# IC3Net/IC3Net

Measured on NVIDIA H100. Metric: agent-env-steps/sec, higher is better.
Workload: dtype f32

## Files before the change

ic3net_b200/_lib.py:

```python
import ctypes as C
import os

import torch

_HERE = os.path.dirname(os.path.abspath(__file__))
LIB_PATH = os.path.join(_HERE, "libic3net_b200.so")

MAX_AGENTS = 32
MAX_HEADS = 4
MAX_HEAD_DIM = 16
MAX_PASSES = 4
CELL_LSTM, CELL_TANH = 0, 1
LSTM_IMG_BYTES = 786432

ERR_EPISODE_DONE = 1
ERR_ROUTE_OVERRUN = 2
ERR_BAD_ACTION = 4
ERR_PIPELINE = 0x100
ERR_FP16_RANGE = 0x200

PP_MODES = {"mixed": 0, "cooperative": 1, "competitive": 2}

_p = C.c_void_p

# ... 52 lines not shown
    _fields_ = [("enc_wT", _p), ("enc_b", _p), ("c_wT", _p), ("c_b", _p), ("lstm_wT", _p), ("lstm_b", _p),
                ("head_w", _p), ("head_b", _p), ("lstm_img", _p), ("bias_cat", _p), ("f_wT", _p), ("f_b", _p), ("flags", _p)]


class PolicyIO(C.Structure):
    _fields_ = [("x", _p), ("h", _p), ("c", _p), ("comm_action", _p), ("alive", _p), ("fresh", _p), ("tick", _p),
                ("draws", _p), ("h_out", _p), ("c_out", _p), ("value", _p), ("logp", _p), ("action", _p),
                ("workspace", _p), ("err", _p), ("pp_env", _p), ("pp_state", _p), ("tj_env", _p), ("tj_state", _p),
                ("x_table", _p), ("defer_heads", C.c_int32), ("pass_index", C.c_int32)]


class BpttPlan(C.Structure):
    _fields_ = [("cfg", C.POINTER(PolicyCfg)), ("w", C.POINTER(PolicyPacked)), ("pp_env", C.POINTER(PPCfg)),
                ("tj_env", C.POINTER(TJCfg)), ("x_table", _p), ("value_coeff", C.c_float), ("entr", C.c_float),
                ("workspace", _p)]


class BpttStepIO(C.Structure):
    _fields_ = [("t", C.c_int32), ("reserved0", C.c_int32), ("h_prev", _p), ("c_prev", _p), ("h_new", _p), ("fresh", _p), ("comm", _p), ("alive", _p), ("cut", _p),
                ("pp_loc", _p), ("tj_loc", _p), ("tj_alive", _p), ("tj_last_act", _p), ("tj_route_id", _p),
                ("logp", _p), ("action", _p), ("value", _p), ("ret", _p), ("adv", _p), ("alive_post", _p),
                ("valid", _p), ("dh", _p), ("dc", _p), ("err", _p)]


_PTR = C.c_void_p
SYMBOLS = {
    "ic3_version": (C.c_char_p, []),
    "ic3_strerror": (C.c_char_p, [C.c_int]),
    "ic3_launch_count": (C.c_uint64, []),
    "ic3_pp_reset": (C.c_int, [C.POINTER(PPCfg), C.POINTER(PPState), _PTR, _PTR, _PTR]),
    "ic3_pp_step": (C.c_int, [C.POINTER(PPCfg), C.POINTER(PPState), _PTR, C.c_int32, _PTR, _PTR, _PTR,
                              C.POINTER(RolloutIO), _PTR]),
    "ic3_pp_obs": (C.c_int, [C.POINTER(PPCfg), C.POINTER(PPState), _PTR, _PTR]),
    "ic3_tj_reset": (C.c_int, [C.POINTER(TJCfg), C.POINTER(TJState), _PTR, _PTR, _PTR]),
    "ic3_tj_step": (C.c_int, [C.POINTER(TJCfg), C.POINTER(TJState), _PTR, C.c_int32, _PTR, _PTR, _PTR, _PTR,
                              C.POINTER(RolloutIO), _PTR]),
    "ic3_tj_obs": (C.c_int, [C.POINTER(TJCfg), C.POINTER(TJState), _PTR, _PTR]),
    "ic3_policy_pack": (C.c_int, [C.POINTER(PolicyCfg), C.POINTER(PolicyParams), C.POINTER(PolicyPacked), _PTR]),
    "ic3_encoder_dense": (C.c_int, [C.POINTER(PolicyCfg), C.POINTER(PolicyPacked), _PTR, _PTR, _PTR]),
    "ic3_pp_encoder_index": (C.c_int, [C.POINTER(PPCfg), C.POINTER(PPState), C.POINTER(PolicyCfg),
                                       C.POINTER(PolicyPacked), _PTR, _PTR]),
    "ic3_tj_encoder_index": (C.c_int, [C.POINTER(TJCfg), C.POINTER(TJState), C.POINTER(PolicyCfg),
                                       C.POINTER(PolicyPacked), _PTR, _PTR]),
    "ic3_pp_obs_encode": (C.c_int, [C.POINTER(PPCfg), C.POINTER(PPState), C.POINTER(PolicyCfg),
                                    C.POINTER(PolicyPacked), _PTR, _PTR, _PTR]),
    "ic3_tj_obs_encode": (C.c_int, [C.POINTER(TJCfg), C.POINTER(TJState), C.POINTER(PolicyCfg),
                                    C.POINTER(PolicyPacked), _PTR, _PTR, _PTR]),
    "ic3_pp_encoder_table":(C.c_int, [C.POINTER(PPCfg), C.POINTER(PolicyCfg), C.POINTER(PolicyPacked), _PTR, _PTR]),
    "ic3_tj_encoder_table": (C.c_int, [C.POINTER(TJCfg), C.POINTER(PolicyCfg), C.POINTER(PolicyPacked), _PTR, _PTR]),
    "ic3_policy_workspace_bytes": (C.c_uint64, [C.POINTER(PolicyCfg)]),
    "ic3_policy_step": (C.c_int, [C.POINTER(PolicyCfg), C.POINTER(PolicyPacked), C.POINTER(PolicyIO), _PTR]),
    "ic3_policy_partial_ptr": (C.c_void_p, [C.POINTER(PolicyCfg), _PTR]),
    "ic3_policy_step_profile": (C.c_int, [C.POINTER(PolicyCfg), C.POINTER(PolicyPacked), C.POINTER(PolicyIO), _PTR,
                                          C.POINTER(C.c_float)]),
    "ic3_sample_actions": (C.c_int, [C.POINTER(PolicyCfg), _PTR, _PTR, _PTR, _PTR, _PTR]),
    "ic3_returns_scan": (C.c_int, [C.c_int32, C.c_int32, C.c_int32, C.c_float, C.c_float, _PTR, _PTR, _PTR, _PTR,
                                   _PTR]),
    "ic3_bptt_workspace_bytes": (C.c_uint64, [C.POINTER(BpttPlan)]),
    "ic3_bptt_begin": (C.c_int, [C.POINTER(BpttPlan), C.c_float, _PTR]),
    "ic3_bptt_step": (C.c_int, [C.POINTER(BpttPlan), C.POINTER(BpttStepIO), _PTR]),
    "ic3_bptt_prepare": (C.c_int, [C.POINTER(BpttPlan), C.POINTER(BpttStepIO), _PTR]),
    "ic3_bptt_finish": (C.c_int, [C.POINTER(BpttPlan), C.POINTER(PolicyParams), C.POINTER(PolicyParams), _PTR, _PTR]),
    "ic3_stat_reduce": (C.c_int, [C.c_int32, C.c_int32, _PTR, _PTR, _PTR, _PTR, _PTR, _PTR, _PTR, _PTR]),
    "ic3_rmsprop_step": (C.c_int, [C.c_int64, C.c_float, C.c_float, C.c_float, C.c_float, _PTR, _PTR, _PTR, _PTR]),
}

_lib = None


def load():
# ... 45 lines not shown
```

ic3net_b200/csrc/ic3_common.cuh:

```cuda
#pragma once
#include <cuda_runtime.h>
#include <stdint.h>

#include "../../include/ic3net_b200.h"

#define IC3_FULL_MASK 0xffffffffu
#define IC3_ENV_WARPS 8

__host__ __device__ __forceinline__ int ic3_pp_agents(const ic3_pp_cfg& c) { return c.N + (c.enemy_comm != 0 ? 1 : 0); }

extern unsigned long long g_ic3_launches;

#define IC3_LAUNCH_CHECK()                         \
  do {                                             \
    ++g_ic3_launches;                              \
    cudaError_t _e = cudaGetLastError();           \
    if (_e != cudaSuccess) return (int)_e;         \
  } while (0)

#define IC3_LAUNCH_RC(expr)                                   \
  do {                                                        \
    ++g_ic3_launches;                                         \
    cudaError_t _e = (expr);                                  \
    if (_e == cudaSuccess) _e = cudaGetLastError();           \
    if (_e != cudaSuccess) return (int)_e;                    \
  } while (0)

__device__ __forceinline__ void ic3_pdl_trigger() { asm volatile("griddepcontrol.launch_dependents;" ::: "memory"); }
__device__ __forceinline__ void ic3_pdl_wait() { asm volatile("griddepcontrol.wait;" ::: "memory"); }

bool ic3_pdl_enabled();

template <typename... KArgs, typename... Args>
inline cudaError_t ic3_launch_pdl(void (*kern)(KArgs...), dim3 grid, dim3 block, size_t smem, cudaStream_t s, Args... args) {
  cudaLaunchConfig_t lc{};
  lc.gridDim = grid;
  lc.blockDim = block;
  lc.dynamicSmemBytes = smem;
  lc.stream = s;
  cudaLaunchAttribute at[1];
// ... 64 lines not shown
```

ic3net_b200/csrc/policy_internal.h:

```cpp
#pragma once
#include <cuda_runtime.h>

#include "../../include/ic3net_b200.h"

uint64_t ic3_tc_workspace_bytes(const ic3_policy_cfg* cfg);
int ic3_tc_pack(const ic3_policy_cfg* cfg, const ic3_policy_params* p, const ic3_policy_packed* out, cudaStream_t s);
int ic3_tc_policy_step(const ic3_policy_cfg* cfg, const ic3_policy_packed* w, const ic3_policy_io* io, cudaStream_t s);
#define IC3_DISPATCH_H(Hval, CALL)          \
  switch (Hval) {                           \
    case 32: { constexpr int HH = 32; return CALL; }   \
    case 64: { constexpr int HH = 64; return CALL; }   \
    case 128: { constexpr int HH = 128; return CALL; } \
    default: return IC3_E_UNSUPPORTED;      \
  }

int ic3_encoder_check(const ic3_policy_cfg* cfg, const ic3_policy_packed* w);
int ic3_pp_layout_check(const ic3_pp_cfg* env, const ic3_policy_cfg* cfg);
int ic3_tj_layout_check(const ic3_tj_cfg* env, const ic3_policy_cfg* cfg);
```

ic3net_b200/csrc/policy_tc.cu:

```cuda
#include "policy_tc_kernels.cuh"


constexpr int TC_TILE_PAD = 8;

static int launch_lstm(const ic3_policy_cfg* cfg, const ic3_policy_io* io, const ic3_policy_packed* w, const __half* a_img,
                       int ntiles_pad, size_t smem, int nout, float* partial, cudaStream_t s) {
  static int max_ctas = 0;
  auto kern = lstm_tc_kernel;
  if (max_ctas == 0) {
    cudaError_t e = cudaFuncSetAttribute(kern, cudaFuncAttributeMaxDynamicSharedMemorySize, (int)smem);
    if (e != cudaSuccess) return (int)e;
    int per_sm = 0, dev = 0, nsm = 0;
    e = cudaOccupancyMaxActiveBlocksPerMultiprocessor(&per_sm, kern, TC_P_THREADS, smem);
    if (e == cudaSuccess) e = cudaGetDevice(&dev);
    if (e == cudaSuccess) e = cudaDeviceGetAttribute(&nsm, cudaDevAttrMultiProcessorCount, dev);
    if (e != cudaSuccess || per_sm <= 0) return e != cudaSuccess ? (int)e : IC3_E_RANGE;
    max_ctas = per_sm * nsm;
  }
  const int nitems = 2 * ntiles_pad;
  cudaLaunchConfig_t lc{};
  lc.gridDim = dim3(nitems < max_ctas ? nitems : max_ctas);
  lc.blockDim = dim3(TC_P_THREADS);
  lc.dynamicSmemBytes = smem;
  lc.stream = s;
  cudaLaunchAttribute la[1];
  la[0].id = cudaLaunchAttributeProgrammaticStreamSerialization;
  la[0].val.programmaticStreamSerializationAllowed = 1;
  lc.attrs = la; lc.numAttrs = ic3_pdl_enabled() ? 1 : 0;
  const __half* b_img = reinterpret_cast<const __half*>(w->lstm_img) + (size_t)io->pass_index * B_IMG_HALFS;
  cudaError_t e = cudaLaunchKernelEx(&lc, kern, *cfg, *io, a_img, b_img,
                                     (const float*)w->bias_cat + (size_t)io->pass_index * 4 * TC_H, nitems,
                                     (const float*)w->head_w, nout, partial);
  ++g_ic3_launches;
  return e == cudaSuccess ? IC3_OK : (int)e;
}

// ... 122 lines not shown
    if (src.table) {
      IC3_LAUNCH_RC(ic3_launch_pdl(prep_kernel<XSRC_PP, true>, dim3(2 * ntiles_pad), dim3(PREP_THREADS), prep_T_bytes(cfg->N), s, *cfg, *io, img, src, PrepBwd{}));
    } else {
      static bool cfgd = false;
      if (!cfgd) {
        cudaError_t e = cudaFuncSetAttribute(prep_kernel<XSRC_PP, false>, cudaFuncAttributeMaxDynamicSharedMemorySize, PREP_X_BYTES + (PREP_ROWS + 2) * TC_H * 4);
        if (e != cudaSuccess) return (int)e;
        cfgd = true;
      }
      IC3_LAUNCH_RC(ic3_launch_pdl(prep_kernel<XSRC_PP, false>, dim3(2 * ntiles_pad), dim3(256), PREP_X_BYTES + prep_T_bytes(cfg->N), s, *cfg, *io, img, src, PrepBwd{}));
    }
  } else if (io->tj_env && io->tj_state) {
    const int W = 2 * io->tj_env->vision + 1;
    if (W * W > PREP_MAX_WW || io->tj_env->B != cfg->B || io->tj_env->N != cfg->N) return IC3_E_RANGE;
    if (cfg->O != 2 + W * W * io->tj_env->vocab) return IC3_E_RANGE;
    src.tj = *io->tj_env;
    src.tjs = *io->tj_state;
    if (int lrc = ic3_tj_layout_check(io->tj_env, cfg)) return lrc;
    if (src.table) {
      IC3_LAUNCH_RC(ic3_launch_pdl(prep_kernel<XSRC_TJ, true>, dim3(2 * ntiles_pad), dim3(PREP_THREADS), prep_T_bytes(cfg->N), s, *cfg, *io, img, src, PrepBwd{}));
    } else {
      static bool cfgd = false;
      if (!cfgd) {
        cudaError_t e = cudaFuncSetAttribute(prep_kernel<XSRC_TJ, false>, cudaFuncAttributeMaxDynamicSharedMemorySize, PREP_X_BYTES + (PREP_ROWS + 2) * TC_H * 4);
        if (e != cudaSuccess) return (int)e;
        cfgd = true;
      }
      IC3_LAUNCH_RC(ic3_launch_pdl(prep_kernel<XSRC_TJ, false>, dim3(2 * ntiles_pad), dim3(256), PREP_X_BYTES + prep_T_bytes(cfg->N), s, *cfg, *io, img, src, PrepBwd{}));
    }
  } else {
    return IC3_E_NULL;
  }
  prof_mark(1, s);
  const size_t smem = NSTAGE_P * STAGE_BYTES + 256 + TC_H * HEAD_PAD * sizeof(float) + 4 * TC_H * sizeof(float);
  int nout = 1;
  for (int k = 0; k < cfg->nheads; ++k) nout += cfg->head_dim[k];
  const bool fused_heads = nout <= HEAD_PAD;
  float* partial = fused_heads ? reinterpret_cast<float*>(reinterpret_cast<unsigned char*>(io->workspace) +
                                                           (size_t)ntiles_pad * TC_NCHUNK * A_CHUNK_BYTES)
                               : nullptr;
  const int rc = launch_lstm(cfg, io, w, img, ntiles_pad, smem, nout, partial, s);
  if (rc) return rc;
  prof_mark(2, s);
  if (!last) return IC3_OK;
  if (fused_heads && io->defer_heads) {
    prof_mark(3, s);
    return IC3_OK;
  }
  if (fused_heads) {
    IC3_LAUNCH_RC(ic3_launch_pdl(heads_finish_kernel, dim3((unsigned)((R + 127) / 128)), dim3(128), 0, s, *cfg, *w, *io,
                                 (const float*)partial));
    prof_mark(3, s);
    return IC3_OK;
  }
  const int P = nout <= 8 ? 8 : (nout <= 16 ? 16 : 32);
  const long rows_per_block = 8L * (32 / P);
  const int hgrid = (int)((R + rows_per_block - 1) / rows_per_block);
  if (P == 8) heads_kernel<8><<<hgrid, 256, 0, s>>>(*cfg, *w, *io);
  else if (P == 16) heads_kernel<16><<<hgrid, 256, 0, s>>>(*cfg, *w, *io);
  else heads_kernel<32><<<hgrid, 256, 0, s>>>(*cfg, *w, *io);
  IC3_LAUNCH_CHECK();
  prof_mark(3, s);
  return IC3_OK;
}
```

ic3net_b200/csrc/pp_env.cu:

```cuda
#include <cstring>

#include "encoder_rows.cuh"
#include "ic3_common.cuh"
#include "policy_internal.h"
#include "rollout_tail.cuh"

namespace {

struct PPArgs {
  ic3_pp_cfg cfg;
  ic3_pp_state st;
};

__device__ __forceinline__ void pp_reset_env(const PPArgs& a, int e, int lane) {
  const int N = a.cfg.N, D = a.cfg.dim, need = N + 1;
  const uint32_t ncell = (uint32_t)(D * D);
  const uint32_t epi = a.st.episode[e];
  int mycell = -1, cnt = 0;
  for (uint32_t blk = 0; cnt < need && blk < 4096u; ++blk) {
    const uint4 w = ic3_draw24(a.cfg.seed, a.cfg.env_id0 + (uint32_t)e, epi, IC3_STREAM_PP_RESET, blk);
#pragma unroll
    for (int i = 0; i < 4; ++i) {
      if (cnt < need) {
        const int cand = (int)ic3_pick(ic3_word(w, i), ncell);
// ... 166 lines not shown
    }
    if (obs && lane <= N) {
      s_r[lane] = rr;
      s_c[lane] = cc;
    }
  }
  if (obs == nullptr) return;
  __syncthreads();
  const int W = 2 * a.cfg.vision + 1;
  pp_write_obs<VEC4>(a.cfg, s_r, s_c, s_cell, obs + (size_t)e * NA * W * W * (D * D + 4), keep_l2 != 0);
}

template <int H, bool VEC4>
__global__ void __launch_bounds__(256) pp_obs_encode_kernel(PPArgs a, float* __restrict__ obs,
                                                            const float* __restrict__ wT, const float* __restrict__ bias,
                                                            float* __restrict__ x, bool split, int keep_l2) {
  ic3_pdl_trigger();
  ic3_pdl_wait();
  extern __shared__ uint32_t s_cell[];
  __shared__ int s_r[IC3_MAX_AGENTS + 1], s_c[IC3_MAX_AGENTS + 1];
  const int N = a.cfg.N, D = a.cfg.dim, W = 2 * a.cfg.vision + 1, WW = W * W, V = D * D + 4;
  const int NA = ic3_pp_agents(a.cfg);
  const int e = blockIdx.x, warp = threadIdx.x >> 5, lane = threadIdx.x & 31;
  if (threadIdx.x <= N) {
    const int* l = a.st.loc + ((size_t)e * (N + 1) + threadIdx.x) * 2;
    s_r[threadIdx.x] = l[0];
    s_c[threadIdx.x] = l[1];
  }
  __syncthreads();
  pp_write_obs<VEC4>(a.cfg, s_r, s_c, s_cell, obs + (size_t)e * NA * WW * V, keep_l2 != 0);
  for (int i = warp; i < NA; i += blockDim.x >> 5) {
    const uint32_t* rec = s_cell + i * WW;
    pp_encode_row<H>([rec](int w) { return rec[w]; }, WW, V, wT, bias, split, x + ((size_t)e * NA + i) * H, lane);
  }
}

int pp_check(const ic3_pp_cfg* cfg, const ic3_pp_state* st) {
  if (!cfg || !st) return IC3_E_NULL;
  if (!st->loc || !st->reached || !st->done || !st->success || !st->episode || !st->tick) return IC3_E_NULL;
  if (cfg->B <= 0 || cfg->N <= 0 || cfg->N >= IC3_MAX_AGENTS) return IC3_E_RANGE;
  if (cfg->dim <= 0 || cfg->dim > 181 || cfg->vision < 0 || cfg->vision > 7) return IC3_E_RANGE;
  if (cfg->N + 1 > cfg->dim * cfg->dim) return IC3_E_RANGE;
  if (cfg->mode < 0 || cfg->mode > 2) return IC3_E_RANGE;
  if (cfg->naction != 4 && cfg->naction != 5) return IC3_E_RANGE;
  return IC3_OK;
}

int pp_launch(const ic3_pp_cfg* cfg, const ic3_pp_state* st, const int32_t* act, int act_stride,
              float* reward, float* obs, int32_t* err, const ic3_rollout_io* r, int do_step,
              cudaStream_t s) {
  PPArgs a{*cfg, *st};
  const int W = 2 * cfg->vision + 1;
  const int V = cfg->dim * cfg->dim + 4;
  const int NA = ic3_pp_agents(*cfg);
  const size_t smem = obs ? (size_t)NA * W * W * sizeof(uint32_t) : 0;
  const int threads = obs ? 256 : 32 * IC3_ENV_WARPS;
  const int grid = obs ? cfg->B : (cfg->B + IC3_ENV_WARPS - 1) / IC3_ENV_WARPS;
  const bool vec4 = (V % 4 == 0) && ((reinterpret_cast<uintptr_t>(obs) & 15) == 0);
  RolloutOpt ro = make_rollout_opt(r);
  const int keep = obs && (size_t)cfg->B * NA * W * W * V * sizeof(float) <= IC3_OBS_L2_KEEP_BYTES;
  if (vec4)
    IC3_LAUNCH_RC(ic3_launch_pdl(pp_step_kernel<true>, dim3(grid), dim3(threads), smem, s, a, act, act_stride, reward, obs,
                                 err, ro, do_step, keep));
  else
    IC3_LAUNCH_RC(ic3_launch_pdl(pp_step_kernel<false>, dim3(grid), dim3(threads), smem, s, a, act, act_stride, reward, obs,
                                 err, ro, do_step, keep));
  return IC3_OK;
}

template <int H>
int pp_obs_encode_launch(const ic3_pp_cfg* cfg, const ic3_pp_state* st, const ic3_policy_cfg* pcfg,
                         const ic3_policy_packed* w, float* obs, float* x, cudaStream_t s) {
  PPArgs a{*cfg, *st};
  const int W = 2 * cfg->vision + 1, V = cfg->dim * cfg->dim + 4, NA = ic3_pp_agents(*cfg);
  const size_t smem = (size_t)NA * W * W * sizeof(uint32_t);
  const bool vec4 = (V % 4 == 0) && ((reinterpret_cast<uintptr_t>(obs) & 15) == 0);
  const bool split = pcfg->obs_vocab > 0;
  const int keep = (size_t)cfg->B * NA * W * W * V * sizeof(float) <= IC3_OBS_L2_KEEP_BYTES;
  const float* wT = w->enc_wT;
  const float* b = w->enc_b;
  if (vec4)
    IC3_LAUNCH_RC(ic3_launch_pdl(pp_obs_encode_kernel<H, true>, dim3(cfg->B), dim3(256), smem, s, a, obs, wT, b, x, split,
                                 keep));
  else
    IC3_LAUNCH_RC(ic3_launch_pdl(pp_obs_encode_kernel<H, false>, dim3(cfg->B), dim3(256), smem, s, a, obs, wT, b, x, split,
                                 keep));
  return IC3_OK;
}

}

extern "C" int ic3_pp_reset(const ic3_pp_cfg* cfg, const ic3_pp_state* st, const uint8_t* mask,
                            float* obs, void* stream) {
  int rc = pp_check(cfg, st);
  if (rc) return rc;
  cudaStream_t s = (cudaStream_t)stream;
  PPArgs a{*cfg, *st};
  const int wpb = 4;
  pp_reset_kernel<<<(cfg->B + wpb - 1) / wpb, wpb * 32, 0, s>>>(a, mask);
  IC3_LAUNCH_CHECK();
  if (obs) return pp_launch(cfg, st, nullptr, 0, nullptr, obs, nullptr, nullptr, 0, s);
  return IC3_OK;
}

extern "C" int ic3_pp_step(const ic3_pp_cfg* cfg, const ic3_pp_state* st, const int32_t* act,
                           int32_t act_stride, float* reward, float* obs, int32_t* err,
                           const ic3_rollout_io* r, void* stream) {
  int rc = pp_check(cfg, st);
  if (rc) return rc;
  if (!act || !reward || !err || act_stride < 1) return IC3_E_NULL;
  if (r && (!r->t_ep || !r->fresh || !r->alive_next || (r->hard_attn && (!r->comm_next || !r->action))))
    return IC3_E_NULL;
  return pp_launch(cfg, st, act, act_stride, reward, obs, err, r, 1, (cudaStream_t)stream);
}

extern "C" int ic3_pp_obs(const ic3_pp_cfg* cfg, const ic3_pp_state* st, float* obs, void* stream) {
  int rc = pp_check(cfg, st);
  if (rc) return rc;
  if (!obs) return IC3_E_NULL;
  return pp_launch(cfg, st, nullptr, 0, nullptr, obs, nullptr, nullptr, 0, (cudaStream_t)stream);
}

// ... 15 lines not shown
```

ic3net_b200/csrc/tj_env.cu:

```cuda
#include <cstring>

#include "encoder_rows.cuh"
#include "ic3_common.cuh"
#include "policy_internal.h"
#include "rollout_tail.cuh"

namespace {

struct TJArgs {
  ic3_tj_cfg cfg;
  ic3_tj_state st;
};

__device__ __forceinline__ void tj_reset_env(const TJArgs& a, int e, int lane) {
  const int N = a.cfg.N;
  if (lane < N) {
    const size_t i = (size_t)e * N + lane;
    a.st.loc[i * 2] = 0;
    a.st.loc[i * 2 + 1] = 0;
    a.st.alive[i] = 0;
    a.st.wait[i] = 0;
    a.st.route_id[i] = -1;
    a.st.route_pos[i] = -1;
    a.st.last_act[i] = 0;
// ... 205 lines not shown

template <int H>
__global__ void __launch_bounds__(128) tj_obs_encode_kernel(TJArgs a, float* __restrict__ obs,
                                                            const float* __restrict__ wT, const float* __restrict__ bias,
                                                            float* __restrict__ x, bool split, int keep_l2) {
  ic3_pdl_trigger();
  ic3_pdl_wait();
  extern __shared__ uint32_t s_cell[];
  __shared__ int s_r[IC3_MAX_AGENTS], s_c[IC3_MAX_AGENTS], s_alive[IC3_MAX_AGENTS], s_rid[IC3_MAX_AGENTS],
      s_lact[IC3_MAX_AGENTS];
  const ic3_tj_cfg& cfg = a.cfg;
  const int N = cfg.N, W = 2 * cfg.vision + 1, WW = W * W, V = cfg.vocab;
  const int e = blockIdx.x, warp = threadIdx.x >> 5, lane = threadIdx.x & 31;
  if (threadIdx.x < N) {
    const size_t i = (size_t)e * N + threadIdx.x;
    s_r[threadIdx.x] = a.st.loc[i * 2];
    s_c[threadIdx.x] = a.st.loc[i * 2 + 1];
    s_alive[threadIdx.x] = a.st.alive[i];
    s_rid[threadIdx.x] = a.st.route_id[i];
    s_lact[threadIdx.x] = a.st.last_act[i];
  }
  __syncthreads();
  tj_write_obs(cfg, s_r, s_c, s_alive, s_rid, s_lact, s_cell, obs + (size_t)e * N * (2 + WW * V), keep_l2 != 0);
  for (int i = warp; i < N; i += blockDim.x >> 5) {
    const uint32_t* rec = s_cell + i * WW;
    const bool alive = s_alive[i] != 0;
    const float la = alive ? (float)s_lact[i] : 0.f;
    const float ri = alive ? (float)s_rid[i] / (float)(cfg.npath - 1) : 0.f;
    tj_encode_row<H>(alive, la, ri, [rec](int w) { return rec[w]; }, WW, V, cfg.car_cls, wT, bias, split,
                     x + ((size_t)e * N + i) * H, lane);
  }
}

int tj_check(const ic3_tj_cfg* cfg, const ic3_tj_state* st) {
  if (!cfg || !st) return IC3_E_NULL;
  if (!st->loc || !st->alive || !st->wait || !st->route_id || !st->route_pos || !st->last_act ||
      !st->completed || !st->cars_in_sys || !st->has_failed || !st->tick)
    return IC3_E_NULL;
  if (!cfg->grid || !cfg->route_len || !cfg->route_cells) return IC3_E_NULL;
  if (cfg->B <= 0 || cfg->N <= 0 || cfg->N > IC3_MAX_AGENTS) return IC3_E_RANGE;
  if (cfg->h <= 0 || cfg->w <= 0 || cfg->h > 32767 || cfg->w > 32767) return IC3_E_RANGE;
  if (cfg->vision < 0 || cfg->vision > 7) return IC3_E_RANGE;
  if (cfg->G <= 0 || cfg->P <= 0 || cfg->Lmax <= 0 || cfg->npath < 2 || cfg->vocab <= 0 || cfg->vocab > 65535)
    return IC3_E_RANGE;
  return IC3_OK;
}

int tj_launch(const ic3_tj_cfg* cfg, const ic3_tj_state* st, const int32_t* act, int act_stride,
              const uint32_t* draws, float* reward, float* obs, int32_t* err, const ic3_rollout_io* r,
              int do_step, cudaStream_t s) {
  TJArgs a{*cfg, *st};
  const int W = 2 * cfg->vision + 1;
  const size_t smem = obs ? (size_t)cfg->N * W * W * sizeof(uint32_t) : 0;
  const int threads = obs ? 128 : 32 * IC3_ENV_WARPS;
  const int grid = obs ? cfg->B : (cfg->B + IC3_ENV_WARPS - 1) / IC3_ENV_WARPS;
  RolloutOpt ro = make_rollout_opt(r);
  const int keep = obs && (size_t)cfg->B * cfg->N * (2 + W * W * cfg->vocab) * sizeof(float) <= IC3_OBS_L2_KEEP_BYTES;
  IC3_LAUNCH_RC(ic3_launch_pdl(tj_step_kernel, dim3(grid), dim3(threads), smem, s, a, act, act_stride, draws, reward, obs, err,
                               ro, do_step, keep));
  return IC3_OK;
}

template <int H>
int tj_obs_encode_launch(const ic3_tj_cfg* cfg, const ic3_tj_state* st, const ic3_policy_cfg* pcfg,
                         const ic3_policy_packed* w, float* obs, float* x, cudaStream_t s) {
  TJArgs a{*cfg, *st};
  const int W = 2 * cfg->vision + 1;
  const size_t smem = (size_t)cfg->N * W * W * sizeof(uint32_t);
  const bool split = pcfg->obs_vocab > 0;
  const int keep = (size_t)cfg->B * cfg->N * (2 + W * W * cfg->vocab) * sizeof(float) <= IC3_OBS_L2_KEEP_BYTES;
  IC3_LAUNCH_RC(ic3_launch_pdl(tj_obs_encode_kernel<H>, dim3(cfg->B), dim3(128), smem, s, a, obs, (const float*)w->enc_wT,
                               (const float*)w->enc_b, x, split, keep));
  return IC3_OK;
}

}

extern "C" int ic3_tj_reset(const ic3_tj_cfg* cfg, const ic3_tj_state* st, const uint8_t* mask,
                            float* obs, void* stream) {
  int rc = tj_check(cfg, st);
  if (rc) return rc;
  cudaStream_t s = (cudaStream_t)stream;
  TJArgs a{*cfg, *st};
  const int wpb = 4;
  tj_reset_kernel<<<(cfg->B + wpb - 1) / wpb, wpb * 32, 0, s>>>(a, mask);
  IC3_LAUNCH_CHECK();
  if (obs) return tj_launch(cfg, st, nullptr, 0, nullptr, nullptr, obs, nullptr, nullptr, 0, s);
  return IC3_OK;
}

extern "C" int ic3_tj_step(const ic3_tj_cfg* cfg, const ic3_tj_state* st, const int32_t* act,
                           int32_t act_stride, const uint32_t* draws, float* reward, float* obs,
                           int32_t* err, const ic3_rollout_io* r, void* stream) {
  int rc = tj_check(cfg, st);
  if (rc) return rc;
  if (!act || !reward || !err || act_stride < 1) return IC3_E_NULL;
  if (r && (!r->t_ep || !r->fresh || !r->alive_next || (r->hard_attn && (!r->comm_next || !r->action))))
    return IC3_E_NULL;
  return tj_launch(cfg, st, act, act_stride, draws, reward, obs, err, r, 1, (cudaStream_t)stream);
}

extern "C" int ic3_tj_obs(const ic3_tj_cfg* cfg, const ic3_tj_state* st, float* obs, void* stream) {
  int rc = tj_check(cfg, st);
  if (rc) return rc;
  if (!obs) return IC3_E_NULL;
  return tj_launch(cfg, st, nullptr, 0, nullptr, nullptr, obs, nullptr, nullptr, 0, (cudaStream_t)stream);
}

extern "C" int ic3_tj_obs_encode(const ic3_tj_cfg* env, const ic3_tj_state* st, const ic3_policy_cfg* cfg,
                                 const ic3_policy_packed* w, float* obs, float* x, void* stream) {
// ... 13 lines not shown
```

ic3net_b200/trainer.py:

```python
import ctypes as C
import math
from collections import namedtuple

import torch
import torch.nn.functional as F

from . import _lib
from .optim import FlatRMSprop
from .utils import merge_stat

Transition = namedtuple('Transition', ('state', 'action', 'action_out', 'value', 'episode_mask',
                                       'episode_mini_mask', 'next_state', 'reward', 'misc'))

RolloutBatch = namedtuple('RolloutBatch', ('action', 'logp', 'value', 'reward', 'episode_mask',
                                           'episode_mini_mask', 'alive_mask', 'valid'))


def policy_forward_torch(net, x, h, c, g, n_alive):
    w, cp = net._kernel_weights(), net._cfg_proto
    B, N = g.shape
    H = x.shape[1]
    lstm = cp['cell'] == _lib.CELL_LSTM
    if cp['x_tanh']:
        x = torch.tanh(x)
# ... 13 lines not shown
            gi, gf, gq, go = gates.chunk(4, dim=1)
            c = torch.sigmoid(gf) * c + torch.sigmoid(gi) * torch.tanh(gq)
            hid = torch.sigmoid(go) * torch.tanh(c)
        else:
            hid = torch.tanh(x + F.linear(hid, w['f_w'][ps], w['f_b'][ps]) + cvec)
    value = F.linear(hid, w['value_w'], w['value_b'])
    logps = [F.log_softmax(F.linear(hid, hw, hb), dim=-1) for hw, hb in zip(w['head_w'], w['head_b'])]
    return hid, c, value, logps


class Trainer(object):
    def __init__(self, args, policy_net, env):
        if not hasattr(policy_net, 'packed'):
            raise NotImplementedError("Trainer drives policies that run on the CUDA kernels (CommNetMLP, models.MLP, "
                                      "models.RNN); models.Random has no kernel path")
        self.args = args
        self.policy_net = policy_net
        self.env = env
        self.display = False
        self.last_step = False
        self.optimizer = FlatRMSprop(policy_net.parameters(), lr=args.lrate, alpha=0.97, eps=1e-6)
        self.params = [p for p in self.policy_net.parameters()]
        self.obs_mode = getattr(args, 'obs_mode', 'index')
        self.use_graph = bool(getattr(args, 'use_graph', False))
        self.is_tj = args.env_name == 'traffic_junction'
        self.record_for_grad = bool(getattr(args, 'record_for_grad', False))
        self.grad_window = int(getattr(args, 'grad_window', 40))
        self.grad_impl = getattr(args, 'grad_impl', None) or 'auto'
        self.grad_kernels = False
        self._bptt = None
        self._buf = None
        self._graph = None
        self._graph_key = None
        policy_net.set_obs_layout(*getattr(env.env, 'obs_layout', (0, 0, 0)))
        self.use_xtable = bool(getattr(args, 'encoder_table', True))
        self._xtable = None
        self._xtable_key = None
        if self.record_for_grad and self.grad_impl in ('auto', 'kernels'):
            ok = self._bptt_supported()
            if self.grad_impl == 'kernels' and not ok:
                raise NotImplementedError("grad_impl='kernels' needs the tensor-core policy path (hid_size 128), the "
                                          "per-position encoder table, <= 7 action logits and a small vision window")
            self.grad_kernels = ok
        if self.grad_impl == 'auto':
            self.grad_impl = 'kernels' if self.grad_kernels else 'autograd'

    def _bptt_supported(self):
        e, net = self.env.env, self.policy_net
        W = 2 * e.vision + 1
        if net.policy_impl != 'tc' or not self.use_xtable or W * W > 25 or 1 + sum(self.args.naction_heads) > 8:
            return False
        if getattr(net, 'is_variant', False):
            return False
        if getattr(e, 'obs_layout', (0, 0, 0))[1] == 0:
            return False
        npos = e.obs_positions
        used = npos + ((W * W + 4) if self.is_tj else (2 * W * W + 1))
        return (used + 15) // 16 * 16 <= 512

    def _encoder_table(self, cfg, w):
        e, net = self.env.env, self.policy_net
        if not self.use_xtable or cfg.obs_vocab == 0:
            return None
        key = net._packed_key
        if self._xtable is None:
            self._xtable = torch.empty(e.obs_positions, net.hid_size, device=e.device)
# ... 40 lines not shown
            if self.is_tj:
                b['s_obs'] = z(T, B, N, self.env.observation_dim)
            else:
                b['s_loc'] = z(T, B, e.npredator + 1, 2, dtype=torch.int32)
        self._buf = b
        self._graph = None
        return b

    def _dense_chunks(self, cfg):
        e, b = self.env.env, self._buf
        B, N, O, H = e.nenvs, self.args.nagents, self.env.observation_dim, self.args.hid_size
        key = (B, b['obs'].data_ptr(), b['x'].data_ptr(), cfg.obs_vocab, cfg.seed, cfg.env_id0)
        if getattr(self, '_chunks_key', None) == key:
            return self._chunks
        mb = float(getattr(self.args, 'obs_chunk_mb', 0) or 0)
        per_env = N * O * 4
        nchunk = max(1, -(-B * per_env // int(mb * (1 << 20)))) if mb > 0 else 1
        step = -(-B // nchunk)
        out = []
        for k0 in range(0, B, step):
            k1 = min(B, k0 + step)
            ecfg, est = e.chunk_view(k0, k1)
            ccfg = _lib.PolicyCfg.from_buffer_copy(cfg)
            ccfg.B, ccfg.env_id0 = k1 - k0, cfg.env_id0 + k0
            out.append((ecfg, est, ccfg, b['obs'].data_ptr() + k0 * per_env, b['x'].data_ptr() + k0 * N * H * 4))
        self._chunks, self._chunks_key = out, key
        return out

    def _fused_x(self):
        dense = self.obs_mode == 'dense' or (self.record_for_grad and self.is_tj and not self.grad_kernels)
        W = 2 * self.env.env.vision + 1
        return (not dense) and self.policy_net.policy_impl == 'tc' and W * W <= 25

    def _enqueue(self, T, quota=0):
        b, e, net, args = self._buf, self.env.env, self.policy_net, self.args
        lib = _lib.load()
        B, N = e.nenvs, args.nagents
        nh = len(args.naction_heads)
        cfg = net.policy_cfg(B)
        cfg.seed, cfg.env_id0 = e.cfg.seed, e.cfg.env_id0
        w = net.packed()
        hard = int(bool(args.hard_attn) and bool(args.commnet))
        s = _lib.stream()
        ws, _ = net.workspace(B)
        rec = self.record_for_grad
        gk = rec and self.grad_kernels
        dense = self.obs_mode == 'dense' or (rec and self.is_tj and not gk)
        fused_x = self._fused_x()
        src = {}
        if fused_x:
            src = dict(tj_env=C.addressof(e.cfg), tj_state=C.addressof(e.state)) if self.is_tj else \
                dict(pp_env=C.addressof(e.cfg), pp_state=C.addressof(e.state))
            src['x_table'] = _lib.ptr(self._encoder_table(cfg, w))
        fuse_heads = (net.policy_impl == 'tc' and 1 + sum(args.naction_heads) <= 8 and ws is not None
                      and bool(getattr(args, 'fuse_heads', False)))
        heads_kw = {}
        if fuse_heads:
            hd = (C.c_int32 * _lib.MAX_HEADS)(*(list(args.naction_heads) + [0] * (_lib.MAX_HEADS - nh)))
            heads_kw = dict(head_partial=lib.ic3_policy_partial_ptr(C.byref(cfg), ws.data_ptr()),
                            head_b=net._bufs['head_b'].data_ptr(), head_dim=hd)
        snap = {}
        if rec:
            snap = dict(snap_T=T, snap_fresh=b['s_fresh'].data_ptr(), snap_comm=b['s_comm'].data_ptr(),
                        snap_alive=b['s_alive'].data_ptr(), snap_tep=b['s_tep'].data_ptr())
            if not self.is_tj:
                snap['snap_pp_loc'] = b['s_loc'].data_ptr()
            elif gk:
                snap.update(snap_tj_loc=b['s_tjloc'].data_ptr(), snap_tj_alive=b['s_tjalive'].data_ptr(),
                            snap_tj_last_act=b['s_tjlast'].data_ptr(), snap_tj_route_id=b['s_tjroute'].data_ptr())
        for t in range(T):
            if rec:
                if t == 0:
                    b['s_fresh'][0].copy_(b['fresh'])
                    b['s_comm'][0].copy_(b['comm'])
                    b['s_alive'][0].copy_(b['alive'])
                    b['s_tep'][0].copy_(b['t_ep'])
                    if not self.is_tj:
                        b['s_loc'][0].copy_(e.loc)
                    elif gk:
                        b['s_tjloc'][0].copy_(e.car_loc)
                        b['s_tjalive'][0].copy_(e.alive_mask)
                        b['s_tjlast'][0].copy_(e.car_last_act)
                        b['s_tjroute'][0].copy_(e.route_id)
                if not gk and t % self.grad_window == 0:
                    b['ck_h'][t // self.grad_window].copy_(b['h'])
                    b['ck_c'][t // self.grad_window].copy_(b['c'])
            if dense:
                obs_enc = lib.ic3_tj_obs_encode if self.is_tj else lib.ic3_pp_obs_encode
                for ecfg, est, ccfg, o_ptr, x_ptr in self._dense_chunks(cfg):
                    _lib.check(obs_enc(C.byref(ecfg), C.byref(est), C.byref(ccfg), C.byref(w), o_ptr, x_ptr, s))
                if rec and self.is_tj:
                    b['s_obs'][t].copy_(b['obs'])
            elif fused_x:
                pass
            elif self.is_tj:
                _lib.check(lib.ic3_tj_encoder_index(C.byref(e.cfg), C.byref(e.state), C.byref(cfg), C.byref(w),
                                                    b['x'].data_ptr(), s))
            else:
                _lib.check(lib.ic3_pp_encoder_index(C.byref(e.cfg), C.byref(e.state), C.byref(cfg), C.byref(w),
                                                    b['x'].data_ptr(), s))
            hin, cin = (b['rec_h'][t], b['rec_c'][t]) if gk else (b['h'], b['c'])
            hout, cout = (b['rec_h'][t + 1], b['rec_c'][t + 1]) if gk else (b['h'], b['c'])
            io = _lib.PolicyIO(x=None if fused_x else b['x'].data_ptr(), h=hin.data_ptr(), c=cin.data_ptr(),
                               comm_action=b['comm'].data_ptr() if hard else None, alive=b['alive'].data_ptr(),
                               fresh=b['fresh'].data_ptr(), tick=e.tick.data_ptr(), draws=None,
                               h_out=hout.data_ptr(), c_out=cout.data_ptr(), value=b['value'][t].data_ptr(),
                               logp=b['logp'][t].data_ptr(), action=b['action'][t].data_ptr(),
                               workspace=_lib.ptr(ws), err=b['err'].data_ptr(), defer_heads=int(fuse_heads), **src)
            _lib.check(lib.ic3_policy_step(C.byref(cfg), C.byref(w), C.byref(io), s))
            if fuse_heads:
                heads_kw.update(head_value=b['value'][t].data_ptr(), head_logp=b['logp'][t].data_ptr())
            r = _lib.RolloutIO(t=t, max_steps=args.max_steps, nheads=nh, hard_attn=hard,
                               comm_action_one=int(bool(args.comm_action_one)),
                               last=int(t == T - 1 and quota <= 0), batch_size=int(quota),
                               halted=b['halted'].data_ptr(), rec_valid=b['valid'].data_ptr(), **snap, **heads_kw,
                               action=b['action'][t].data_ptr(), t_ep=b['t_ep'].data_ptr(),
                               fresh=b['fresh'].data_ptr(), comm_next=b['comm'].data_ptr(),
                               alive_next=b['alive'].data_ptr(), rec_reward=b['reward'].data_ptr(),
                               rec_episode_mask=b['emask'].data_ptr(), rec_mini_mask=b['mini'].data_ptr(),
                               rec_alive=b['ralive'].data_ptr(), stat_reward=b['stat_reward'].data_ptr(),
                               stat_comm=b['stat_comm'].data_ptr(), stat_success=b['stat_success'].data_ptr(),
                               stat_episodes=b['stat_episodes'].data_ptr(), stat_steps=b['stat_steps'].data_ptr())
            if self.is_tj:
                _lib.check(lib.ic3_tj_step(C.byref(e.cfg), C.byref(e.state), b['action'][t].data_ptr(), nh, None,
                                           b['step_reward'].data_ptr(), None, b['err'].data_ptr(), C.byref(r), s))
            else:
                _lib.check(lib.ic3_pp_step(C.byref(e.cfg), C.byref(e.state), b['action'][t].data_ptr(), nh,
                                           b['step_reward'].data_ptr(), None, b['err'].data_ptr(), C.byref(r), s))

    def _episode_boundary(self, epoch):
        e, b = self.env.env, self._buf
        if self.is_tj:
            e.reset(epoch, want_obs=False)
        else:
            e.reset(want_obs=False)
        for k in ('stat_reward', 'stat_comm', 'stat_success', 'stat_episodes', 'stat_steps', 't_ep', 'halted'):
            b[k].zero_()
        b['fresh'].fill_(1)

    def rollout(self, T, epoch=0, quota=0):
        e = self.env.env
        if self._buf is None or self._buf['T'] != T:
            self._alloc(T)
        b = self._buf
# ... 333 lines not shown
```

include/ic3net_b200.h:

```cpp
#ifndef IC3NET_B200_H
#define IC3NET_B200_H

#include <stdint.h>

#ifdef __cplusplus
extern "C" {
#endif

#define IC3_MAX_AGENTS 32
#define IC3_MAX_HEADS 4
#define IC3_MAX_HEAD_DIM 16

enum {
  IC3_OK = 0,
  IC3_E_NULL = -1,
  IC3_E_RANGE = -2,
  IC3_E_UNSUPPORTED = -3
};

enum {
  IC3_ERR_EPISODE_DONE = 1,
  IC3_ERR_ROUTE_OVERRUN = 2,
  IC3_ERR_BAD_ACTION = 4,
  IC3_ERR_PIPELINE = 0x100,
// ... 45 lines not shown
  uint8_t* rec_alive;
  float* stat_reward;
  float* stat_comm;
  int32_t* stat_success;
  int32_t* stat_episodes;
  int32_t* stat_steps;
  int32_t batch_size;
  int32_t reserved0;
  uint8_t* halted;
  uint8_t* rec_valid;
  int32_t snap_T;
  int32_t reserved1;
  uint8_t* snap_fresh;
  uint8_t* snap_comm;
  uint8_t* snap_alive;
  int32_t* snap_tep;
  int32_t* snap_pp_loc;
  int32_t* snap_tj_loc;
  uint8_t* snap_tj_alive;
  uint8_t* snap_tj_last_act;
  int32_t* snap_tj_route_id;
  const float* head_partial;
  const float* head_b;
  float* head_value;
  float* head_logp;
  int32_t head_dim[IC3_MAX_HEADS];
} ic3_rollout_io;

int ic3_pp_reset(const ic3_pp_cfg* cfg, const ic3_pp_state* st, const uint8_t* mask,
                 float* obs, void* stream);
int ic3_pp_step(const ic3_pp_cfg* cfg, const ic3_pp_state* st, const int32_t* act, int32_t act_stride,
                float* reward, float* obs, int32_t* err, const ic3_rollout_io* r, void* stream);
int ic3_pp_obs(const ic3_pp_cfg* cfg, const ic3_pp_state* st, float* obs, void* stream);

typedef struct {
  int32_t B, N, vision;
  int32_t h, w;
  int32_t G, P, Lmax;
  int32_t outside_cls;
  int32_t car_cls;
  int32_t vocab;
  int32_t npath;
  uint32_t spawn_thr;
  uint32_t env_id0;
  uint64_t seed;
  const int32_t* grid;
  const int32_t* route_len;
  const int32_t* route_cells;
} ic3_tj_cfg;

typedef struct {
  int32_t* loc;
  uint8_t* alive;
  int32_t* wait;
  int32_t* route_id;
  int32_t* route_pos;
  uint8_t* last_act;
  uint8_t* completed;
  int32_t* cars_in_sys;
  uint8_t* has_failed;
  uint32_t* tick;
} ic3_tj_state;

int ic3_tj_reset(const ic3_tj_cfg* cfg, const ic3_tj_state* st, const uint8_t* mask,
                 float* obs, void* stream);
int ic3_tj_step(const ic3_tj_cfg* cfg, const ic3_tj_state* st, const int32_t* act, int32_t act_stride,
                const uint32_t* draws, float* reward, float* obs, int32_t* err,
                const ic3_rollout_io* r, void* stream);
int ic3_tj_obs(const ic3_tj_cfg* cfg, const ic3_tj_state* st, float* obs, void* stream);

typedef struct {
  int32_t B, N, H, O;
  int32_t nheads;
  int32_t head_dim[IC3_MAX_HEADS];
  int32_t hard_attn;
  int32_t comm_avg;
  int32_t comm_mask_zero;
  uint32_t env_id0;
  uint64_t seed;
  int32_t obs_off, obs_vocab, obs_ncount;
  int32_t cell, passes, x_tanh, h_from_x;
  int32_t reserved0;
} ic3_policy_cfg;

enum { IC3_CELL_LSTM = 0, IC3_CELL_TANH = 1 };
#define IC3_MAX_PASSES 4

typedef struct {
  const float* encoder_w;
  const float* encoder_b;
  const float* c_w;
  const float* c_b;
  const float* w_ih;
  const float* w_hh;
  const float* b_ih;
  const float* b_hh;
  const float* value_w;
  const float* value_b;
  const float* head_w[IC3_MAX_HEADS];
  const float* head_b[IC3_MAX_HEADS];
  const float* c_w_pass[IC3_MAX_PASSES];
  const float* c_b_pass[IC3_MAX_PASSES];
// ... 136 lines not shown
```

Baseline: 92.55 million.

## Overlap dense observation writes with LSTM policy step on a side stream

In dense observation mode with large observation buffers, the observation write is moved to a side stream. It runs concurrently with the policy step, which now reads from the fused env-state encoder path instead of the dense encode. New bounded obs-writer kernels get a grid sized from occupancy calculations so they fit in the SM resources left beside the LSTM kernel, with grid-stride loops and prefetching of agent locations. The aim is to hide the cost of writing observations behind the recurrent compute, at the price of cross-stream syncs and possible contention with the LSTM kernel.

```diff
diff --git a/ic3net_b200/_lib.py b/ic3net_b200/_lib.py
--- a/ic3net_b200/_lib.py
+++ b/ic3net_b200/_lib.py
@@ -108,10 +108,12 @@
     "ic3_pp_step": (C.c_int, [C.POINTER(PPCfg), C.POINTER(PPState), _PTR, C.c_int32, _PTR, _PTR, _PTR,
                               C.POINTER(RolloutIO), _PTR]),
     "ic3_pp_obs": (C.c_int, [C.POINTER(PPCfg), C.POINTER(PPState), _PTR, _PTR]),
+    "ic3_pp_obs_bounded": (C.c_int, [C.POINTER(PPCfg), C.POINTER(PPState), _PTR, _PTR]),
     "ic3_tj_reset": (C.c_int, [C.POINTER(TJCfg), C.POINTER(TJState), _PTR, _PTR, _PTR]),
     "ic3_tj_step": (C.c_int, [C.POINTER(TJCfg), C.POINTER(TJState), _PTR, C.c_int32, _PTR, _PTR, _PTR, _PTR,
                               C.POINTER(RolloutIO), _PTR]),
     "ic3_tj_obs": (C.c_int, [C.POINTER(TJCfg), C.POINTER(TJState), _PTR, _PTR]),
+    "ic3_tj_obs_bounded": (C.c_int, [C.POINTER(TJCfg), C.POINTER(TJState), _PTR, _PTR]),
     "ic3_policy_pack": (C.c_int, [C.POINTER(PolicyCfg), C.POINTER(PolicyParams), C.POINTER(PolicyPacked), _PTR]),
     "ic3_encoder_dense": (C.c_int, [C.POINTER(PolicyCfg), C.POINTER(PolicyPacked), _PTR, _PTR, _PTR]),
     "ic3_pp_encoder_index": (C.c_int, [C.POINTER(PPCfg), C.POINTER(PPState), C.POINTER(PolicyCfg),
diff --git a/ic3net_b200/csrc/ic3_common.cuh b/ic3net_b200/csrc/ic3_common.cuh
--- a/ic3net_b200/csrc/ic3_common.cuh
+++ b/ic3net_b200/csrc/ic3_common.cuh
@@ -6,6 +6,8 @@
 
 #define IC3_FULL_MASK 0xffffffffu
 #define IC3_ENV_WARPS 8
+#define IC3_OBS_WRITER_THREADS 256
+#define IC3_OBS_WRITER_MIN_CTAS (65536 / (IC3_OBS_WRITER_THREADS * 64))
 
 __host__ __device__ __forceinline__ int ic3_pp_agents(const ic3_pp_cfg& c) { return c.N + (c.enemy_comm != 0 ? 1 : 0); }
 
diff --git a/ic3net_b200/csrc/policy_internal.h b/ic3net_b200/csrc/policy_internal.h
--- a/ic3net_b200/csrc/policy_internal.h
+++ b/ic3net_b200/csrc/policy_internal.h
@@ -6,6 +6,7 @@
 uint64_t ic3_tc_workspace_bytes(const ic3_policy_cfg* cfg);
 int ic3_tc_pack(const ic3_policy_cfg* cfg, const ic3_policy_params* p, const ic3_policy_packed* out, cudaStream_t s);
 int ic3_tc_policy_step(const ic3_policy_cfg* cfg, const ic3_policy_packed* w, const ic3_policy_io* io, cudaStream_t s);
+int ic3_grid_beside_lstm(const void* kern, int threads, size_t smem, int nwork, int* grid);
 #define IC3_DISPATCH_H(Hval, CALL)          \
   switch (Hval) {                           \
     case 32: { constexpr int HH = 32; return CALL; }   \
diff --git a/ic3net_b200/csrc/policy_tc.cu b/ic3net_b200/csrc/policy_tc.cu
--- a/ic3net_b200/csrc/policy_tc.cu
+++ b/ic3net_b200/csrc/policy_tc.cu
@@ -1,7 +1,54 @@
+#include <algorithm>
+
 #include "policy_tc_kernels.cuh"
 
 
 constexpr int TC_TILE_PAD = 8;
+constexpr size_t LSTM_SMEM_BYTES = NSTAGE_P * STAGE_BYTES + 256 + TC_H * HEAD_PAD * sizeof(float) + 4 * TC_H * sizeof(float);
+
+static int ctas_beside_lstm(const void* kern, int threads, size_t smem, int* per_sm, int* nsm) {
+  cudaFuncAttributes la, ka;
+  cudaError_t e = cudaFuncGetAttributes(&la, lstm_tc_kernel);
+  if (e == cudaSuccess) e = cudaFuncGetAttributes(&ka, kern);
+  int dev = 0, regs = 0, smem_sm = 0, reserved = 0, thr_sm = 0, blk_sm = 0;
+  if (e == cudaSuccess) e = cudaGetDevice(&dev);
+  if (e == cudaSuccess) e = cudaDeviceGetAttribute(nsm, cudaDevAttrMultiProcessorCount, dev);
+  if (e == cudaSuccess) e = cudaDeviceGetAttribute(&regs, cudaDevAttrMaxRegistersPerMultiprocessor, dev);
+  if (e == cudaSuccess) e = cudaDeviceGetAttribute(&smem_sm, cudaDevAttrMaxSharedMemoryPerMultiprocessor, dev);
+  if (e == cudaSuccess) e = cudaDeviceGetAttribute(&reserved, cudaDevAttrReservedSharedMemoryPerBlock, dev);
+  if (e == cudaSuccess) e = cudaDeviceGetAttribute(&thr_sm, cudaDevAttrMaxThreadsPerMultiProcessor, dev);
+  if (e == cudaSuccess) e = cudaDeviceGetAttribute(&blk_sm, cudaDevAttrMaxBlocksPerMultiprocessor, dev);
+  if (e != cudaSuccess) return (int)e;
+  auto cta_regs = [](const cudaFuncAttributes& a, int nthr) { return ((a.numRegs * 32 + 255) / 256 * 256) * ((nthr + 31) / 32); };
+  const long free_regs = (long)regs - cta_regs(la, TC_P_THREADS);
+  const long free_smem = (long)smem_sm - (long)(LSTM_SMEM_BYTES + la.sharedSizeBytes + reserved);
+  long n = free_regs / cta_regs(ka, threads);
+  n = std::min(n, free_smem / (long)(smem + ka.sharedSizeBytes + reserved));
+  n = std::min(n, (long)(thr_sm - TC_P_THREADS) / threads);
+  n = std::min(n, (long)blk_sm - 1);
+  *per_sm = n > 1 ? (int)n : 1;
+  return IC3_OK;
+}
+
+int ic3_grid_beside_lstm(const void* kern, int threads, size_t smem, int nwork, int* grid) {
+  struct Entry { const void* kern; int threads; size_t smem; int ctas; };
+  static Entry cache[8];
+  static int ncache = 0;
+  int ctas = 0;
+  for (int i = 0; i < ncache; ++i)
+    if (cache[i].kern == kern && cache[i].threads == threads && cache[i].smem == smem) ctas = cache[i].ctas;
+  if (ctas == 0) {
+    cudaError_t e = cudaFuncSetAttribute(kern, cudaFuncAttributePreferredSharedMemoryCarveout, cudaSharedmemCarveoutMaxShared);
+    if (e != cudaSuccess) return (int)e;
+    int per_sm = 0, nsm = 0;
+    const int rc = ctas_beside_lstm(kern, threads, smem, &per_sm, &nsm);
+    if (rc) return rc;
+    ctas = per_sm * nsm;
+    if (ncache < 8) cache[ncache++] = Entry{kern, threads, smem, ctas};
+  }
+  *grid = nwork < ctas ? nwork : ctas;
+  return IC3_OK;
+}
 
 static int launch_lstm(const ic3_policy_cfg* cfg, const ic3_policy_io* io, const ic3_policy_packed* w, const __half* a_img,
                        int ntiles_pad, size_t smem, int nout, float* partial, cudaStream_t s) {
@@ -190,7 +237,7 @@
     return IC3_E_NULL;
   }
   prof_mark(1, s);
-  const size_t smem = NSTAGE_P * STAGE_BYTES + 256 + TC_H * HEAD_PAD * sizeof(float) + 4 * TC_H * sizeof(float);
+  const size_t smem = LSTM_SMEM_BYTES;
   int nout = 1;
   for (int k = 0; k < cfg->nheads; ++k) nout += cfg->head_dim[k];
   const bool fused_heads = nout <= HEAD_PAD;
diff --git a/ic3net_b200/csrc/pp_env.cu b/ic3net_b200/csrc/pp_env.cu
--- a/ic3net_b200/csrc/pp_env.cu
+++ b/ic3net_b200/csrc/pp_env.cu
@@ -222,6 +222,38 @@
   for (int i = warp; i < NA; i += blockDim.x >> 5) {
     const uint32_t* rec = s_cell + i * WW;
     pp_encode_row<H>([rec](int w) { return rec[w]; }, WW, V, wT, bias, split, x + ((size_t)e * NA + i) * H, lane);
+  }
+}
+
+template <bool VEC4>
+__global__ void __launch_bounds__(IC3_OBS_WRITER_THREADS, IC3_OBS_WRITER_MIN_CTAS)
+    pp_obs_writer_kernel(PPArgs a, float* __restrict__ obs, int keep_l2) {
+  ic3_pdl_trigger();
+  ic3_pdl_wait();
+  extern __shared__ uint32_t s_cell[];
+  __shared__ int s_r[IC3_MAX_AGENTS + 1], s_c[IC3_MAX_AGENTS + 1];
+  const int N = a.cfg.N, W = 2 * a.cfg.vision + 1, B = a.cfg.B;
+  const size_t per_env = (size_t)ic3_pp_agents(a.cfg) * W * W * (a.cfg.dim * a.cfg.dim + 4);
+  const int k = threadIdx.x;
+  int r = 0, c = 0;
+  if (k <= N && (int)blockIdx.x < B) {
+    const int* l = a.st.loc + ((size_t)blockIdx.x * (N + 1) + k) * 2;
+    r = l[0];
+    c = l[1];
+  }
+  for (int e = blockIdx.x; e < B; e += gridDim.x) {
+    if (k <= N) {
+      s_r[k] = r;
+      s_c[k] = c;
+      if (e + (int)gridDim.x < B) {
+        const int* l = a.st.loc + ((size_t)(e + gridDim.x) * (N + 1) + k) * 2;
+        r = l[0];
+        c = l[1];
+      }
+    }
+    __syncthreads();
+    pp_write_obs<VEC4>(a.cfg, s_r, s_c, s_cell, obs + (size_t)e * per_env, keep_l2 != 0);
+    __syncthreads();
   }
 }
 
@@ -278,6 +310,29 @@
   return IC3_OK;
 }
 
+template <bool VEC4>
+int pp_obs_bounded_launch(const ic3_pp_cfg* cfg, const ic3_pp_state* st, float* obs, cudaStream_t s) {
+  PPArgs a{*cfg, *st};
+  const int W = 2 * cfg->vision + 1, V = cfg->dim * cfg->dim + 4, NA = ic3_pp_agents(*cfg);
+  const size_t smem = (size_t)NA * W * W * sizeof(uint32_t);
+  const int keep = (size_t)cfg->B * NA * W * W * V * sizeof(float) <= IC3_OBS_L2_KEEP_BYTES;
+  auto kern = pp_obs_writer_kernel<VEC4>;
+  int grid = 0;
+  const int rc = ic3_grid_beside_lstm((const void*)kern, IC3_OBS_WRITER_THREADS, smem, cfg->B, &grid);
+  if (rc) return rc;
+  IC3_LAUNCH_RC(ic3_launch_pdl(kern, dim3(grid), dim3(IC3_OBS_WRITER_THREADS), smem, s, a, obs, keep));
+  return IC3_OK;
+}
+
+}
+
+extern "C" int ic3_pp_obs_bounded(const ic3_pp_cfg* cfg, const ic3_pp_state* st, float* obs, void* stream) {
+  int rc = pp_check(cfg, st);
+  if (rc) return rc;
+  if (!obs) return IC3_E_NULL;
+  const bool vec4 = ((cfg->dim * cfg->dim + 4) % 4 == 0) && ((reinterpret_cast<uintptr_t>(obs) & 15) == 0);
+  return vec4 ? pp_obs_bounded_launch<true>(cfg, st, obs, (cudaStream_t)stream)
+              : pp_obs_bounded_launch<false>(cfg, st, obs, (cudaStream_t)stream);
 }
 
 extern "C" int ic3_pp_reset(const ic3_pp_cfg* cfg, const ic3_pp_state* st, const uint8_t* mask,
diff --git a/ic3net_b200/csrc/tj_env.cu b/ic3net_b200/csrc/tj_env.cu
--- a/ic3net_b200/csrc/tj_env.cu
+++ b/ic3net_b200/csrc/tj_env.cu
@@ -261,6 +261,42 @@
   }
 }
 
+__global__ void __launch_bounds__(IC3_OBS_WRITER_THREADS, IC3_OBS_WRITER_MIN_CTAS)
+    tj_obs_writer_kernel(TJArgs a, float* __restrict__ obs, int keep_l2) {
+  ic3_pdl_trigger();
+  ic3_pdl_wait();
+  extern __shared__ uint32_t s_cell[];
+  __shared__ int s_r[IC3_MAX_AGENTS], s_c[IC3_MAX_AGENTS], s_alive[IC3_MAX_AGENTS], s_rid[IC3_MAX_AGENTS],
+      s_lact[IC3_MAX_AGENTS];
+  const ic3_tj_cfg& cfg = a.cfg;
+  const int N = cfg.N, W = 2 * cfg.vision + 1, B = cfg.B;
+  const size_t per_env = (size_t)N * (2 + W * W * cfg.vocab);
+  const int k = threadIdx.x;
+  int r = 0, c = 0, alive = 0, rid = 0, lact = 0;
+  auto load = [&](int e) {
+    const size_t i = (size_t)e * N + k;
+    r = a.st.loc[i * 2];
+    c = a.st.loc[i * 2 + 1];
+    alive = a.st.alive[i];
+    rid = a.st.route_id[i];
+    lact = a.st.last_act[i];
+  };
+  if (k < N && (int)blockIdx.x < B) load(blockIdx.x);
+  for (int e = blockIdx.x; e < B; e += gridDim.x) {
+    if (k < N) {
+      s_r[k] = r;
+      s_c[k] = c;
+      s_alive[k] = alive;
+      s_rid[k] = rid;
+      s_lact[k] = lact;
+      if (e + (int)gridDim.x < B) load(e + gridDim.x);
+    }
+    __syncthreads();
+    tj_write_obs(cfg, s_r, s_c, s_alive, s_rid, s_lact, s_cell, obs + (size_t)e * per_env, keep_l2 != 0);
+    __syncthreads();
+  }
+}
+
 int tj_check(const ic3_tj_cfg* cfg, const ic3_tj_state* st) {
   if (!cfg || !st) return IC3_E_NULL;
   if (!st->loc || !st->alive || !st->wait || !st->route_id || !st->route_pos || !st->last_act ||
@@ -305,6 +341,22 @@
 
 }
 
+extern "C" int ic3_tj_obs_bounded(const ic3_tj_cfg* cfg, const ic3_tj_state* st, float* obs, void* stream) {
+  int rc = tj_check(cfg, st);
+  if (rc) return rc;
+  if (!obs) return IC3_E_NULL;
+  TJArgs a{*cfg, *st};
+  const int W = 2 * cfg->vision + 1;
+  const size_t smem = (size_t)cfg->N * W * W * sizeof(uint32_t);
+  const int keep = (size_t)cfg->B * cfg->N * (2 + W * W * cfg->vocab) * sizeof(float) <= IC3_OBS_L2_KEEP_BYTES;
+  int grid = 0;
+  rc = ic3_grid_beside_lstm((const void*)tj_obs_writer_kernel, IC3_OBS_WRITER_THREADS, smem, cfg->B, &grid);
+  if (rc) return rc;
+  IC3_LAUNCH_RC(ic3_launch_pdl(tj_obs_writer_kernel, dim3(grid), dim3(IC3_OBS_WRITER_THREADS), smem,
+                               (cudaStream_t)stream, a, obs, keep));
+  return IC3_OK;
+}
+
 extern "C" int ic3_tj_reset(const ic3_tj_cfg* cfg, const ic3_tj_state* st, const uint8_t* mask,
                             float* obs, void* stream) {
   int rc = tj_check(cfg, st);
diff --git a/ic3net_b200/trainer.py b/ic3net_b200/trainer.py
--- a/ic3net_b200/trainer.py
+++ b/ic3net_b200/trainer.py
@@ -69,6 +69,7 @@
         self._buf = None
         self._graph = None
         self._graph_key = None
+        self._side = None
         policy_net.set_obs_layout(*getattr(env.env, 'obs_layout', (0, 0, 0)))
         self.use_xtable = bool(getattr(args, 'encoder_table', True))
         self._xtable = None
@@ -175,6 +176,17 @@
         W = 2 * self.env.env.vision + 1
         return (not dense) and self.policy_net.policy_impl == 'tc' and W * W <= 25
 
+    OVERLAP_MIN_OBS_BYTES = 8 << 20
+
+    def _overlap_obs(self):
+        if self.obs_mode != 'dense' or (self.record_for_grad and self.is_tj and not self.grad_kernels):
+            return False
+        e = self.env.env
+        if e.nenvs * self.args.nagents * self.env.observation_dim * 4 < self.OVERLAP_MIN_OBS_BYTES:
+            return False
+        W = 2 * e.vision + 1
+        return self.policy_net.policy_impl == 'tc' and W * W <= 25
+
     def _enqueue(self, T, quota=0):
         b, e, net, args = self._buf, self.env.env, self.policy_net, self.args
         lib = _lib.load()
@@ -189,12 +201,19 @@
         rec = self.record_for_grad
         gk = rec and self.grad_kernels
         dense = self.obs_mode == 'dense' or (rec and self.is_tj and not gk)
-        fused_x = self._fused_x()
+        overlap = self._overlap_obs()
+        fused_x = self._fused_x() or overlap
         src = {}
         if fused_x:
             src = dict(tj_env=C.addressof(e.cfg), tj_state=C.addressof(e.state)) if self.is_tj else \
                 dict(pp_env=C.addressof(e.cfg), pp_state=C.addressof(e.state))
-            src['x_table'] = _lib.ptr(self._encoder_table(cfg, w))
+            src['x_table'] = None if overlap else _lib.ptr(self._encoder_table(cfg, w))
+        if overlap:
+            main = torch.cuda.current_stream()
+            if self._side is None or self._side.device != main.device:
+                self._side = torch.cuda.Stream(device=main.device)
+            side = self._side
+            obs_write = lib.ic3_tj_obs_bounded if self.is_tj else lib.ic3_pp_obs_bounded
         fuse_heads = (net.policy_impl == 'tc' and 1 + sum(args.naction_heads) <= 8 and ws is not None
                       and bool(getattr(args, 'fuse_heads', False)))
         heads_kw = {}
@@ -228,7 +247,11 @@
                 if not gk and t % self.grad_window == 0:
                     b['ck_h'][t // self.grad_window].copy_(b['h'])
                     b['ck_c'][t // self.grad_window].copy_(b['c'])
-            if dense:
+            if overlap:
+                side.wait_stream(main)
+                for ecfg, est, _, o_ptr, _ in self._dense_chunks(cfg):
+                    _lib.check(obs_write(C.byref(ecfg), C.byref(est), o_ptr, side.cuda_stream))
+            elif dense:
                 obs_enc = lib.ic3_tj_obs_encode if self.is_tj else lib.ic3_pp_obs_encode
                 for ecfg, est, ccfg, o_ptr, x_ptr in self._dense_chunks(cfg):
                     _lib.check(obs_enc(C.byref(ecfg), C.byref(est), C.byref(ccfg), C.byref(w), o_ptr, x_ptr, s))
@@ -253,6 +276,8 @@
             _lib.check(lib.ic3_policy_step(C.byref(cfg), C.byref(w), C.byref(io), s))
             if fuse_heads:
                 heads_kw.update(head_value=b['value'][t].data_ptr(), head_logp=b['logp'][t].data_ptr())
+            if overlap:
+                main.wait_stream(side)
             r = _lib.RolloutIO(t=t, max_steps=args.max_steps, nheads=nh, hard_attn=hard,
                                comm_action_one=int(bool(args.comm_action_one)),
                                last=int(t == T - 1 and quota <= 0), batch_size=int(quota),
diff --git a/include/ic3net_b200.h b/include/ic3net_b200.h
--- a/include/ic3net_b200.h
+++ b/include/ic3net_b200.h
@@ -101,6 +101,7 @@
 int ic3_pp_step(const ic3_pp_cfg* cfg, const ic3_pp_state* st, const int32_t* act, int32_t act_stride,
                 float* reward, float* obs, int32_t* err, const ic3_rollout_io* r, void* stream);
 int ic3_pp_obs(const ic3_pp_cfg* cfg, const ic3_pp_state* st, float* obs, void* stream);
+int ic3_pp_obs_bounded(const ic3_pp_cfg* cfg, const ic3_pp_state* st, float* obs, void* stream);
 
 typedef struct {
   int32_t B, N, vision;
@@ -137,6 +138,7 @@
                 const uint32_t* draws, float* reward, float* obs, int32_t* err,
                 const ic3_rollout_io* r, void* stream);
 int ic3_tj_obs(const ic3_tj_cfg* cfg, const ic3_tj_state* st, float* obs, void* stream);
+int ic3_tj_obs_bounded(const ic3_tj_cfg* cfg, const ic3_tj_state* st, float* obs, void* stream);
 
 typedef struct {
   int32_t B, N, H, O;
```

Result: faster. 100.5 million (median of 6 runs) (+8.6%).
